# ray-project/ray_shuffling_data_loader

Hardware: AMD Instinct MI355X
Metric: shuffled_rows_per_sec (higher is better)
Workload: dtype bf16; 1 GPU; model=shuffling-data-loader + TabularMLP(100-512-256-128-1), global_batch=250000, rows_per_gpu=12500000, num_cols=100, batch_size_per_rank=250000, num_reducers=4, max_concurrent_epochs=2, parallelism=dp1, seed=0, burn_steps=0

## Files before the change

csrc/chain.h:

```cpp
#pragma once

#include <hip/hip_runtime.h>

#include <cstdint>

namespace rsdl {

struct ChainWeights {
  const void* W1;
  const float* b1;
  const void* W2;
  const float* b2;
  const void* W3;
  const float* b3;
  const void* w4;
  const float* b4;
};

struct FwdChainArgs {
  const void* x0s;
  ChainWeights w;
  void* a1t;
  uint32_t* mask1;
  void* a2t;
// ... 6 lines not shown
  int64_t M;
  int pi16, rows;
  int loss;
  bool weighted;
  const float* weight;
  float pos_weight;
};

struct EvalChainArgs {
  const void* x0s;
  ChainWeights w;
  float* pred;
  const float* target;
  float* part;
  int64_t M;
  int rows;
  int task;
  int64_t* hist;
  bool weighted;
  const float* weight;
};

struct BwdChainArgs {
  const void* dy;
  const void* a3;
  const void* mask1;
  const void* mask2;
  const void* w4;
  const void* W3T;
  const void* W2T;
  void* dz1t;
  void* dz2t;
  void* dz3t;
  float* db_part;
  int64_t M;
  int pi16, rows;
};

int64_t fwd_chain_grid(int64_t M, int rows);
void launch_swizzle_x(const void* x, void* out, int64_t M,
                      hipStream_t stream);
void launch_swizzle_xt(const void* x, void* out, int64_t M, int pi16,
                       hipStream_t stream);
void launch_swizzle_x_both(const void* x, void* xs, void* xt, int64_t M,
                           int pi16, hipStream_t stream);
void launch_fwd_chain(const FwdChainArgs& p, hipStream_t stream);
void launch_eval_chain(const EvalChainArgs& p, hipStream_t stream);

int64_t bwd_chain_grid(int64_t M, int rows);
void launch_bwd_chain(const BwdChainArgs& p, hipStream_t stream);

int64_t wgrad_frag_nslabs(int64_t mchunks, int32_t N, int32_t K,
                          int32_t nt_w, int32_t kt_w);
void launch_wgrad_frag(const void* AT, const void* BT, float* dW, int32_t N,
                       int32_t K, int64_t mchunks, int32_t nt_w,
                       int32_t kt_w, hipStream_t stream);
void launch_slab_reduce(const float* part, float* out, int64_t nk,
                        int64_t nslabs, hipStream_t stream);

}
```

csrc/shuffle_ops.cpp:

```cpp

#include <torch/extension.h>

#include <c10/hip/HIPStream.h>
#include <hip/hip_runtime.h>

#include <cmath>
#include <cstdlib>
#include <cstring>
#include <tuple>
#include <vector>

#include "chain.h"
#include "step_glue.h"

namespace rsdl {

enum DType : int32_t {
  DT_F32 = 0,
  DT_F64 = 1,
  DT_I32 = 2,
  DT_I64 = 3,
  DT_F16 = 4,
  DT_BF16 = 5,
  DT_U8 = 6,
// ... 816 lines not shown
              "bwd_chain: dy must be contiguous bf16 [M] or [M,1]");
  auto chk_a = [M](const at::Tensor& a, int64_t n, const char* nm) {
    TORCH_CHECK(a.is_cuda() && a.scalar_type() == at::kBFloat16 &&
                    a.dim() == 2 && a.size(0) == M && a.size(1) == n &&
                    a.is_contiguous(),
                "bwd_chain: ", nm, " must be contiguous bf16 [M,", n, "]");
  };
  chk_a(a3, 128, "a3");
  TORCH_CHECK(mask1.is_cuda() && mask1.scalar_type() == at::kInt &&
                  mask1.is_contiguous() && mask1.numel() == mtiles * 512,
              "bwd_chain: mask1 must be int32 [mtiles,512]");
  TORCH_CHECK(mask2.is_cuda() && mask2.scalar_type() == at::kInt &&
                  mask2.is_contiguous() && mask2.numel() == mtiles * 256,
              "bwd_chain: mask2 must be int32 [mtiles,256]");
  TORCH_CHECK(w4.numel() == 128 && w4.scalar_type() == at::kBFloat16,
              "bwd_chain: w4 must be bf16 [128]");
  TORCH_CHECK(W3.scalar_type() == at::kBFloat16 &&
                  ((W3.size(0) == 128 && W3.size(1) == 256) ||
                   (W3.size(0) == 256 && W3.size(1) == 128)),
              "bwd_chain: W3 must be bf16 [128,256] or W3^T [256,128]");
  TORCH_CHECK(W2.scalar_type() == at::kBFloat16 &&
                  ((W2.size(0) == 256 && W2.size(1) == 512) ||
                   (W2.size(0) == 512 && W2.size(1) == 256)),
              "bwd_chain: W2 must be bf16 [256,512] or W2^T [512,256]");
  auto w4c = w4.contiguous();
  auto W3Ts = (W3.size(0) == 128) ? swizzle_frag_T(W3.contiguous())
                                  : swizzle_frag(W3.contiguous());
  auto W2Ts = (W2.size(0) == 256) ? swizzle_frag_T(W2.contiguous())
                                  : swizzle_frag(W2.contiguous());
  auto bo = run_bwd_chain(dy, a3, mask1, mask2, w4c, W3Ts, W2Ts, pi16,
                          crows);
  auto& dz1t = bo.dz1t;
  auto& dz2t = bo.dz2t;
  auto& dz3t = bo.dz3t;
  auto& db_part = bo.db_part;
  auto db_full = at::zeros({kPartWPad}, dy.options().dtype(at::kFloat));
  launch_slab_reduce(db_part.data_ptr<float>(), db_full.data_ptr<float>(),
                     kPartWPad, db_part.size(0), current_stream());
  auto db = db_full.narrow(0, 0, kPartW);
  auto dw4 = (db.narrow(0, 897, 128) + db.narrow(0, 897 + 128, 128))
                 .reshape({1, 128});
  return {dz1t,
          dz2t,
          dz3t,
          db.narrow(0, 0, 512),
          db.narrow(0, 512, 256),
          db.narrow(0, 512 + 256, 128),
          db.narrow(0, 512 + 256 + 128, 1),
          dw4};
}

at::Tensor run_wgrad_frag(const at::Tensor& AT, const at::Tensor& BT,
                          int64_t N, int64_t K, int64_t mchunks,
                          int64_t nt_w, int64_t kt_w) {
  const int64_t nslabs = wgrad_frag_nslabs(mchunks, (int32_t)N, (int32_t)K,
                                           (int32_t)nt_w, (int32_t)kt_w);
  auto part = at::empty({nslabs, N * K}, AT.options().dtype(at::kFloat));
  launch_wgrad_frag(AT.data_ptr(), BT.data_ptr(), part.data_ptr<float>(),
                    (int32_t)N, (int32_t)K, mchunks, (int32_t)nt_w,
                    (int32_t)kt_w, current_stream());
  return part;
}

}
at::Tensor swizzle_xt_bf16(const at::Tensor& x, bool pi16) {
  check_x("swizzle_xt", x);
  const int64_t M = x.size(0);
  const int64_t mtiles = std::max<int64_t>((M + 31) / 32, 1);
  auto out = at::empty({4 * mtiles * 2 * 512}, x.options());
  if (M > 0) {
    launch_swizzle_xt(x.data_ptr(), out.data_ptr(), M, pi16 ? 1 : 0,
                      current_stream());
  }
  return out;
}

at::Tensor wgrad_frag_bf16(const at::Tensor& AT, const at::Tensor& BT,
                           int64_t N, int64_t K, int64_t mchunks,
                           int64_t nt_w, int64_t kt_w) {
  TORCH_CHECK(AT.is_cuda() && AT.scalar_type() == at::kBFloat16 &&
                  AT.is_contiguous() && BT.is_cuda() &&
                  BT.scalar_type() == at::kBFloat16 && BT.is_contiguous(),
              "wgrad_frag: inputs must be contiguous bf16 on GPU");
  TORCH_CHECK(AT.numel() == (N / 32) * mchunks * 512,
              "wgrad_frag: AT numel mismatch");
  TORCH_CHECK(BT.numel() == (K / 32) * mchunks * 512,
              "wgrad_frag: BT numel mismatch");
  TORCH_CHECK((nt_w == 2 && kt_w == 4) || (nt_w == 1 && kt_w == 8) ||
                  (nt_w == 1 && kt_w == 4),
              "wgrad_frag: unsupported tile config");
  TORCH_CHECK(N % (nt_w * 128) == 0 && K % (kt_w * 32) == 0,
              "wgrad_frag: N/K not divisible by block shape");
  auto dW = at::zeros({N, K}, AT.options().dtype(at::kFloat));
  if (mchunks > 0) {
    auto part = run_wgrad_frag(AT, BT, N, K, mchunks, nt_w, kt_w);
    const int64_t nslabs = part.size(0);
    launch_slab_reduce(part.data_ptr<float>(), dW.data_ptr<float>(),
                       N * K, nslabs, current_stream());
  }
  return dW;
}

namespace {

void check_master(const std::vector<at::Tensor>& w, const char* who) {
  TORCH_CHECK(w.size() == 4, who, ": weights must be [W1, W2, W3, w4]");
  const int64_t shp[4][2] = {{512, 100}, {256, 512}, {128, 256}, {1, 128}};
  for (int i = 0; i < 4; i++) {
    TORCH_CHECK(w[i].is_cuda() && w[i].scalar_type() == at::kFloat &&
                    w[i].is_contiguous() &&
                    w[i].numel() == shp[i][0] * shp[i][1] &&
                    (i == 3 || (w[i].dim() == 2 && w[i].size(0) == shp[i][0])),
                who, ": weight ", i, " must be contiguous fp32 [", shp[i][0],
                ",", shp[i][1], "] on GPU");
    TORCH_CHECK(reinterpret_cast<uintptr_t>(w[i].data_ptr()) % 16 == 0,
                who, ": weight ", i, " must be 16-byte aligned");
  }
}

struct PrepOut {
  at::Tensor W1s, W2s, W3s, W2Ts, W3Ts, w4b, tgt;
};

PrepOut run_step_prep(const std::vector<at::Tensor>& w,
                      const c10::optional<at::Tensor>& target,
                      const c10::optional<std::vector<at::Tensor>>& bufs) {
  check_master(w, "step_prep");
  const int64_t numel[6] = {512 * 112, 256 * 512, 128 * 256,
                            256 * 512, 128 * 256, 128};
  at::Tensor o[6];
  auto bf = w[0].options().dtype(at::kBFloat16);
  if (bufs.has_value()) {
    TORCH_CHECK(bufs->size() == 6, "step_prep: need six output buffers");
  }
  for (int i = 0; i < 6; i++) {
    if (bufs.has_value()) {
      o[i] = (*bufs)[i];
      TORCH_CHECK(o[i].is_cuda() && o[i].scalar_type() == at::kBFloat16 &&
                      o[i].is_contiguous() && o[i].numel() == numel[i] &&
                      reinterpret_cast<uintptr_t>(o[i].data_ptr()) % 16 == 0,
                  "step_prep: output buffer ", i,
                  " must be contiguous aligned bf16 with ", numel[i],
                  " elements");
    } else {
      o[i] = at::empty({numel[i]}, bf);
    }
  }
  PrepOut r{o[0], o[1], o[2], o[3], o[4], o[5], at::Tensor()};
  StepPrepArgs p{};
  p.W1 = w[0].data_ptr<float>();
  p.W2 = w[1].data_ptr<float>();
  p.W3 = w[2].data_ptr<float>();
  p.w4 = w[3].data_ptr<float>();
// ... 69 lines not shown
  }
  auto loss = at::empty({}, f32);
  StepFinArgs p{};
  p.part1 = part1.data_ptr<float>();
  p.part2 = part2.data_ptr<float>();
  p.part3 = part3.data_ptr<float>();
  p.db_part = db_part.data_ptr<float>();
  p.loss_part = loss_part.data_ptr<float>();
  p.ns1 = part1.size(0);
  p.ns2 = part2.size(0);
  p.ns3 = part3.size(0);
  p.db_rows = db_part.size(0);
  p.loss_n = loss_part.numel();
  p.M = M;
  p.dw1 = o[0].data_ptr<float>();
  p.dw2 = o[1].data_ptr<float>();
  p.dw3 = o[2].data_ptr<float>();
  p.dw4 = o[3].data_ptr<float>();
  p.db1 = o[4].data_ptr<float>();
  p.db2 = o[5].data_ptr<float>();
  p.db3 = o[6].data_ptr<float>();
  p.db4 = o[7].data_ptr<float>();
  p.loss = loss.data_ptr<float>();
  launch_step_finalize(p, current_stream());
  return {loss, o[0], o[1], o[2], o[3], o[4], o[5], o[6], o[7]};
}

}

std::vector<at::Tensor> step_prep(
    const std::vector<at::Tensor>& weights,
    const c10::optional<at::Tensor>& target,
    const c10::optional<std::vector<at::Tensor>>& outs) {
  auto r = run_step_prep(weights, target, outs);
  std::vector<at::Tensor> v = {r.W1s, r.W2s, r.W3s, r.W2Ts, r.W3Ts, r.w4b};
  if (target.has_value()) v.push_back(r.tgt);
  return v;
}

std::vector<at::Tensor> step_finalize(
    const at::Tensor& part1, const at::Tensor& part2,
    const at::Tensor& part3, const at::Tensor& db_part,
    const at::Tensor& loss_part, int64_t M,
    const c10::optional<std::vector<at::Tensor>>& outs) {
  return run_step_finalize(part1, part2, part3, db_part, loss_part, M, outs);
}

std::vector<at::Tensor> fused_step_bf16(
    const at::Tensor& x, const at::Tensor& target,
    const std::vector<at::Tensor>& weights,
    const std::vector<at::Tensor>& biases, bool pi16,
    const c10::optional<std::vector<at::Tensor>>& outs, int64_t rows,
    int64_t loss, const c10::optional<at::Tensor>& weight,
    double pos_weight) {
  const int crows = chain_rows(rows);
  const int closs = chain_loss(loss, "fused_step", "loss");
  const HeadWeights hw =
      head_weights("fused_step", x, weight, pos_weight, closs);
  check_x("fused_step", x);
  const int64_t M = x.size(0);
  TORCH_CHECK(M > 0, "fused_step: empty batch");
  TORCH_CHECK(target.numel() == M, "fused_step: target size mismatch");
  check_biases("fused_step", biases);
  auto pr = run_step_prep(weights, target, c10::nullopt);
  const int64_t mchunks = 2 * ((M + 31) / 32);
  c10::optional<at::Tensor> xt =
      at::empty({4 * mchunks * 512}, x.options());
  auto f = run_fwd_chain(x, pr.W1s, pr.W2s, pr.W3s, pr.w4b, biases[0],
                         biases[1], biases[2], biases[3], &pr.tgt, xt, pi16,
                         crows, closs, hw);
  auto b = run_bwd_chain(f.dyb, f.a3, f.mask1, f.mask2, pr.w4b, pr.W3Ts,
                         pr.W2Ts, pi16, crows);
  const char* st = std::getenv("RSDL_WGRAD_SMALL_TILES");
  const int64_t kt23 = (st != nullptr && std::strcmp(st, "1") == 0) ? 4 : 8;
  auto p1 = run_wgrad_frag(b.dz1t, *xt, 512, 128, mchunks, 2, 4);
  auto p2 = run_wgrad_frag(b.dz2t, f.a1t, 256, 512, mchunks, 1, kt23);
  auto p3 = run_wgrad_frag(b.dz3t, f.a2t, 128, 256, mchunks, 1, kt23);
  return run_step_finalize(p1, p2, p3, b.db_part, f.loss_part, M, outs);
}

std::tuple<c10::optional<at::Tensor>, c10::optional<at::Tensor>>
eval_chain_bf16(const at::Tensor& x, const std::vector<at::Tensor>& Wstage,
                const std::vector<at::Tensor>& biases,
                const c10::optional<at::Tensor>& target,
                const c10::optional<at::Tensor>& pred_out, bool want_pred,
                int64_t rows, int64_t task,
                const c10::optional<at::Tensor>& hist,
                const c10::optional<at::Tensor>& weight) {
  const int crows = chain_rows(rows);
  const int ctask = chain_loss(task, "eval_chain", "task");
  check_x("eval_chain", x);
  const int64_t M = x.size(0);
  TORCH_CHECK(Wstage.size() == 4,
              "eval_chain: Wstage must be [W1s, W2s, W3s, w4b]");
  const int64_t wn[4] = {512 * 112, 256 * 512, 128 * 256, 128};
  for (int i = 0; i < 4; i++) {
    TORCH_CHECK(Wstage[i].is_cuda() &&
                    Wstage[i].scalar_type() == at::kBFloat16 &&
                    Wstage[i].is_contiguous() && Wstage[i].numel() == wn[i] &&
                    Wstage[i].get_device() == x.get_device() &&
                    reinterpret_cast<uintptr_t>(Wstage[i].data_ptr()) % 16 ==
                        0,
                "eval_chain: staged weight ", i,
                " must be contiguous aligned bf16 with ", wn[i],
                " elements on x's GPU");
  }
  check_biases("eval_chain", biases, x.get_device());
  const bool with_pred = want_pred || pred_out.has_value();
  TORCH_CHECK(with_pred || target.has_value(),
              "eval_chain: nothing to compute (no target, no predictions)");
  at::Tensor tgt, pred, part;
  if (target.has_value()) {
    TORCH_CHECK(target->is_cuda() &&
                    target->get_device() == x.get_device() &&
                    (target->scalar_type() == at::kFloat ||
                     target->scalar_type() == at::kDouble),
                "eval_chain: target must be fp32 or fp64 on x's GPU");
    TORCH_CHECK(target->numel() == M, "eval_chain: target size mismatch");
    tgt = target->reshape({-1}).to(at::kFloat).contiguous();
  }
  if (pred_out.has_value()) {
    TORCH_CHECK(pred_out->is_cuda() &&
                    pred_out->get_device() == x.get_device() &&
                    pred_out->scalar_type() == at::kFloat &&
                    pred_out->is_contiguous() && pred_out->numel() == M,
                "eval_chain: pred_out must be contiguous fp32 with ", M,
                " elements on x's GPU");
    pred = *pred_out;
  } else if (with_pred) {
    pred = at::empty({M}, x.options().dtype(at::kFloat));
// ... 50 lines not shown
                     int64_t M) {
  TORCH_CHECK(part.is_cuda() && part.scalar_type() == at::kFloat &&
                  part.is_contiguous() && part.dim() == 2 &&
                  (part.size(1) == 4 || part.size(1) == 8) &&
                  reinterpret_cast<uintptr_t>(part.data_ptr()) % 16 == 0,
              "eval_accumulate: part must be contiguous aligned fp32 [n,4] "
              "(or [n,8], weighted) on GPU");
  const bool wide = part.size(1) == 8;
  TORCH_CHECK(acc.is_cuda() && acc.scalar_type() == at::kDouble &&
                  acc.is_contiguous() && acc.numel() == (wide ? 6 : 5) &&
                  acc.get_device() == part.get_device(),
              "eval_accumulate: acc must be contiguous fp64 [",
              wide ? 6 : 5, "] on part's GPU");
  TORCH_CHECK(M >= 0, "eval_accumulate: M must not be negative");
  launch_eval_accumulate(part.data_ptr<float>(), part.size(0), M,
                         acc.data_ptr<double>(), wide ? 5 : 4,
                         current_stream());
}

}

PYBIND11_MODULE(TORCH_EXTENSION_NAME, m) {
  m.doc() = "MI355X (gfx950) fused shuffle kernels";
  m.def("gather_rows", &rsdl::gather_rows, "row gather of packed rows",
        py::arg("src"), py::arg("perm"));
  m.def("gather_rows_out", &rsdl::gather_rows_out, py::arg("src"),
        py::arg("perm"), py::arg("dst"));
  m.def("unpack_permute", &rsdl::unpack_permute, py::arg("packed"),
        py::arg("perm"), py::arg("outs"), py::arg("packed_offsets"),
        py::arg("src_dtype_codes"));
  m.def("unpack_permute_affine", &rsdl::unpack_permute_affine,
        py::arg("packed"), py::arg("perm"), py::arg("outs"),
        py::arg("packed_offsets"), py::arg("src_dtype_codes"),
        py::arg("aff_table"), py::arg("aff_base"),
        py::arg("nan_fill") = c10::nullopt);
  m.def("column_stats", &rsdl::column_stats, py::arg("packed"),
        py::arg("packed_offsets"), py::arg("src_dtype_codes"),
        py::arg("numels"));
  m.def("pack_columns", &rsdl::pack_columns, py::arg("cols"),
        py::arg("packed_offsets"), py::arg("packed_dtype_codes"),
        py::arg("row_stride"), py::arg("perm") = c10::nullopt);
  m.def("pack_columns_tiled", &rsdl::pack_columns_tiled, py::arg("cols"),
        py::arg("packed_offsets"), py::arg("packed_dtype_codes"),
        py::arg("row_stride"), py::arg("out") = c10::nullopt);
  m.def("partition_build_perm", &rsdl::partition_build_perm, py::arg("dest"),
        py::arg("num_dests"));
  m.def("wgrad_bf16", &rsdl::wgrad_bf16, py::arg("dy"), py::arg("x"),
        py::arg("with_bias") = true);
  m.def("relu_bwd_bias", &rsdl::relu_bwd_bias, py::arg("dy"), py::arg("y"));
  m.def("swizzle_xt_bf16", &rsdl::swizzle_xt_bf16, py::arg("x"),
        py::arg("pi16") = false);
  m.def("wgrad_frag_bf16", &rsdl::wgrad_frag_bf16, py::arg("AT"),
        py::arg("BT"), py::arg("N"), py::arg("K"), py::arg("mchunks"),
        py::arg("nt_w"), py::arg("kt_w"));
  m.def("fwd_chain_bf16", &rsdl::fwd_chain_bf16, py::arg("x"),
        py::arg("W1"), py::arg("b1"), py::arg("W2"), py::arg("b2"),
        py::arg("W3"), py::arg("b3"), py::arg("w4"), py::arg("b4"),
        py::arg("target") = c10::nullopt,
        py::arg("xt_out") = c10::nullopt, py::arg("pi16") = false,
        py::arg("rows") = 0, py::arg("loss") = 0,
        py::arg("weight") = c10::nullopt, py::arg("pos_weight") = 1.0);
  m.def("bwd_chain_bf16", &rsdl::bwd_chain_bf16, py::arg("dy"),
        py::arg("a3"), py::arg("mask1"), py::arg("mask2"), py::arg("w4"),
        py::arg("W3"), py::arg("W2"), py::arg("pi16") = false,
        py::arg("rows") = 0);
  m.def("step_prep", &rsdl::step_prep, py::arg("weights"),
        py::arg("target") = c10::nullopt, py::arg("outs") = c10::nullopt);
  m.def("step_finalize", &rsdl::step_finalize, py::arg("part1"),
        py::arg("part2"), py::arg("part3"), py::arg("db_part"),
        py::arg("loss_part"), py::arg("M"), py::arg("outs") = c10::nullopt);
  m.def("fused_step_bf16", &rsdl::fused_step_bf16, py::arg("x"),
        py::arg("target"), py::arg("weights"), py::arg("biases"),
        py::arg("pi16") = false, py::arg("outs") = c10::nullopt,
        py::arg("rows") = 0, py::arg("loss") = 0,
        py::arg("weight") = c10::nullopt, py::arg("pos_weight") = 1.0);
  m.def("eval_chain_bf16", &rsdl::eval_chain_bf16, py::arg("x"),
        py::arg("Wstage"), py::arg("biases"),
        py::arg("target") = c10::nullopt, py::arg("pred_out") = c10::nullopt,
        py::arg("want_pred") = true, py::arg("rows") = 0,
        py::arg("task") = 0, py::arg("hist") = c10::nullopt,
        py::arg("weight") = c10::nullopt);
  m.def("eval_accumulate", &rsdl::eval_accumulate, py::arg("part"),
        py::arg("acc"), py::arg("M"));
  m.attr("LOSS_MSE") = (int)rsdl::kLossMse;
  m.attr("LOSS_BCE") = (int)rsdl::kLossBce;
  m.attr("HEAD_WEIGHTS") = 1;
  m.attr("DT_F32") = (int)rsdl::DT_F32;
  m.attr("DT_F64") = (int)rsdl::DT_F64;
  m.attr("DT_I32") = (int)rsdl::DT_I32;
  m.attr("DT_I64") = (int)rsdl::DT_I64;
  m.attr("DT_F16") = (int)rsdl::DT_F16;
  m.attr("DT_BF16") = (int)rsdl::DT_BF16;
  m.attr("DT_U8") = (int)rsdl::DT_U8;
}
```

csrc/wgrad_frag.hip:

```cpp

#include <hip/hip_runtime.h>
#include <hip/hip_bf16.h>

#include <cstdint>
#include <cstdlib>

#include "chain.h"

namespace rsdl {

typedef __attribute__((__vector_size__(8 * sizeof(short)))) short wf_bf16x8;
typedef __attribute__((__vector_size__(16 * sizeof(float)))) float wf_f32x16;

template <int NT_W, int KT_W, int MIN_WAVES = 2, int SCHED = 0>
__global__ void __launch_bounds__(256, MIN_WAVES) wgrad_frag_kernel(
    const short* __restrict__ AT, const short* __restrict__ BT,
    float* __restrict__ dW,
    int32_t N, int32_t K, int64_t mchunks, int32_t nblk_n, int32_t nblk_k,
    int64_t nslabs, int64_t chunks_per_slab) {
  const int32_t NBLK = (nblk_n < 0 ? -nblk_n : nblk_n) * nblk_k;
  int64_t slab;
  int32_t blk;
  if (nblk_n < 0) {
    nblk_n = -nblk_n;
// ... 92 lines not shown
    if (i + 2 < iters) WF_MFMA(a2, b2);
    if (i + 3 < iters) WF_MFMA(a0, b0);
  } else if (SCHED2) {
    WF_LOAD(a0, b0, 0);
    WF_LOAD(a1, b1, 1);
    while (i + 4 <= iters) {
      WF_FENCE();
      WF_MFMA(a0, b0);
      WF_FENCE();
      WF_LOAD(a0, b0, i + 2);
      WF_FENCE();
      WF_MFMA(a1, b1);
      WF_FENCE();
      WF_LOAD(a1, b1, i + 3);
      WF_FENCE();
      i += 2;
    }
    if (i + 2 < iters) WF_LOAD(a2, b2, i + 2);
    if (i < iters) WF_MFMA(a0, b0);
    if (i + 1 < iters) WF_MFMA(a1, b1);
    if (i + 2 < iters) WF_MFMA(a2, b2);
  } else {
    while (i + 3 <= iters) {
      WF_LOAD(a2, b2, i + 2);
      WF_MFMA(a0, b0);
      if (i + 3 < iters) WF_LOAD(a0, b0, i + 3);
      WF_MFMA(a1, b1);
      if (i + 4 < iters) WF_LOAD(a1, b1, i + 4);
      WF_MFMA(a2, b2);
      i += 3;
    }
    if (i < iters) WF_MFMA(a0, b0);
    if (i + 1 < iters) WF_MFMA(a1, b1);
  }
#undef WF_LOAD
#undef WF_MFMA
#undef WF_FENCE

  float* part = dW + slab * (int64_t)N * K;
  #pragma unroll
  for (int nt = 0; nt < NT_W; nt++) {
    #pragma unroll
    for (int kt = 0; kt < KT_W; kt++) {
      const int32_t k = (kt0 + kt) * 32 + (lane & 31);
      #pragma unroll
      for (int reg = 0; reg < 16; reg++) {
        const int32_t n = (nt0 + nt) * 32 + (reg & 3) + 8 * (reg >> 2) +
                          4 * (lane >> 5);
        part[(int64_t)n * K + k] = acc[nt][kt][reg];
      }
    }
  }
}

typedef __attribute__((__vector_size__(4 * sizeof(float)))) float wf_f32x4;
template <int SCHED = 0>
__global__ void __launch_bounds__(256) slab_reduce_kernel(
    const float* __restrict__ part, float* __restrict__ out, int64_t nk4,
    int64_t nslabs, int64_t s1) {
  const int64_t i = (int64_t)blockIdx.x * 256 + threadIdx.x;
  if (i >= nk4) return;
  const int64_t lo = (int64_t)blockIdx.y * s1;
  const int64_t hi = min(lo + s1, nslabs);
  wf_f32x4 s0 = {0.f, 0.f, 0.f, 0.f}, s1v = s0, s2 = s0, s3 = s0;
  int64_t sl = lo;
  if (SCHED) {
    wf_f32x4 la[4], lb[4];
#define SR_LOAD(buf, base)                                                 \
  {                                                                        \
    _Pragma("unroll") for (int j = 0; j < 4; j++) {                        \
      buf[j] = *reinterpret_cast<const wf_f32x4*>(                         \
          part + (((base) + j) * nk4 + i) * 4);                            \
    }                                                                      \
  }
#define SR_ACC(buf)                                                        \
  {                                                                        \
    s0 += buf[0];                                                          \
    s1v += buf[1];                                                         \
    s2 += buf[2];                                                          \
    s3 += buf[3];                                                          \
  }
    if (sl + 4 <= hi) {
      SR_LOAD(la, sl);
      while (sl + 12 <= hi) {
        SR_LOAD(lb, sl + 4);
        __builtin_amdgcn_sched_barrier(0);
        SR_ACC(la);
        __builtin_amdgcn_sched_barrier(0);
        SR_LOAD(la, sl + 8);
        __builtin_amdgcn_sched_barrier(0);
        SR_ACC(lb);
        __builtin_amdgcn_sched_barrier(0);
        sl += 8;
      }
      if (sl + 8 <= hi) {
        SR_LOAD(lb, sl + 4);
        SR_ACC(la);
        SR_ACC(lb);
        sl += 8;
      } else {
        SR_ACC(la);
        sl += 4;
      }
    }
#undef SR_LOAD
#undef SR_ACC
// ... 10 lines not shown
      s0 += l0;
      s1v += l1;
      s2 += l2;
      s3 += l3;
    }
  }
  for (; sl < hi; sl++) {
    s0 += *reinterpret_cast<const wf_f32x4*>(part + (sl * nk4 + i) * 4);
  }
  const wf_f32x4 s = (s0 + s1v) + (s2 + s3);
  float* o = out + i * 4;
  unsafeAtomicAdd(&o[0], s[0]);
  unsafeAtomicAdd(&o[1], s[1]);
  unsafeAtomicAdd(&o[2], s[2]);
  unsafeAtomicAdd(&o[3], s[3]);
}

void launch_slab_reduce(const float* part, float* out, int64_t nk,
                        int64_t nslabs, hipStream_t stream) {
  const int64_t nk4 = nk / 4;
  const int64_t gx = (nk4 + 255) / 256;
  int64_t nsplit = (512 + gx - 1) / gx;
  if (nsplit > nslabs) nsplit = nslabs;
  const int64_t s1 = (nslabs + nsplit - 1) / nsplit;
  nsplit = (nslabs + s1 - 1) / s1;
  static bool sched = [] {
    const char* e = std::getenv("RSDL_WGRAD_SCHED");
    return e && e[0] == '1';
  }();
  auto kern = sched ? slab_reduce_kernel<1> : slab_reduce_kernel<0>;
  hipLaunchKernelGGL(kern,
                     dim3((uint32_t)gx, (uint32_t)nsplit), dim3(256), 0,
                     stream, part, out, nk4, nslabs, s1);
}

static int64_t frag_target(int32_t K, int32_t nt_w) {
  static int64_t env_target = [] {
    const char* e = std::getenv("RSDL_WGRAD_WGS");
    return e ? atoll(e) : 0;
  }();
  if (env_target > 0) return env_target;
  return (nt_w == 2) ? 256 : (K >= 512 ? 512 : 256);
}

int64_t wgrad_frag_nslabs(int64_t mchunks, int32_t N, int32_t K,
                          int32_t nt_w, int32_t kt_w) {
  const int32_t nblk = (N / (nt_w * 128)) * (K / (kt_w * 32));
  int64_t nslabs = (frag_target(K, nt_w) + nblk - 1) / nblk;
  if (nslabs > mchunks) nslabs = mchunks;
  const int64_t cps = (mchunks + nslabs - 1) / nslabs;
  return (mchunks + cps - 1) / cps;
}

void launch_wgrad_frag(const void* AT, const void* BT, float* dW, int32_t N,
                       int32_t K, int64_t mchunks, int32_t nt_w,
                       int32_t kt_w, hipStream_t stream) {
  const int32_t nblk_n = N / (nt_w * 128);
  const int32_t nblk_k = K / (kt_w * 32);
  const int32_t nblk = nblk_n * nblk_k;
  int64_t target = frag_target(K, nt_w);
  int64_t nslabs = (target + nblk - 1) / nblk;
  if (nslabs > mchunks) nslabs = mchunks;
  const int64_t chunks_per_slab = (mchunks + nslabs - 1) / nslabs;
  nslabs = (mchunks + chunks_per_slab - 1) / chunks_per_slab;
  static bool linear = std::getenv("RSDL_WGRAD_LINEAR") != nullptr;
  static bool sched = [] {
    const char* e = std::getenv("RSDL_WGRAD_SCHED");
    return e && e[0] == '1';
  }();
  const int64_t grid =
      linear ? nslabs * nblk : ((nslabs + 7) / 8) * 8 * nblk;
  const int32_t nb_n = linear ? -nblk_n : nblk_n;
  if (nt_w == 2 && kt_w == 4) {
    auto kern = sched ? wgrad_frag_kernel<2, 4, 2, 1>
                      : wgrad_frag_kernel<2, 4>;
    hipLaunchKernelGGL(kern, dim3((uint32_t)grid),
                       dim3(256), 0, stream,
                       reinterpret_cast<const short*>(AT),
                       reinterpret_cast<const short*>(BT), dW, N, K, mchunks,
                       nb_n, nblk_k, nslabs, chunks_per_slab);
  } else if (nt_w == 1 && kt_w == 8) {
    auto kern = sched ? wgrad_frag_kernel<1, 8, 2, 1>
                      : wgrad_frag_kernel<1, 8>;
    hipLaunchKernelGGL(kern, dim3((uint32_t)grid),
                       dim3(256), 0, stream,
                       reinterpret_cast<const short*>(AT),
                       reinterpret_cast<const short*>(BT), dW, N, K, mchunks,
                       nb_n, nblk_k, nslabs, chunks_per_slab);
  } else if (nt_w == 1 && kt_w == 4) {
    auto kern = sched ? wgrad_frag_kernel<1, 4, 3, 1>
                      : wgrad_frag_kernel<1, 4, 3>;
    hipLaunchKernelGGL(kern, dim3((uint32_t)grid),
                       dim3(256), 0, stream,
                       reinterpret_cast<const short*>(AT),
                       reinterpret_cast<const short*>(BT), dW, N, K, mchunks,
                       nb_n, nblk_k, nslabs, chunks_per_slab);
  }
}

}
```

ray_shuffling_data_loader_amd/models/fused_step.py:

```python

import os
from typing import Tuple

import torch

from ray_shuffling_data_loader_amd.models.mlp import TabularMLP

_PI16 = os.environ.get("RSDL_PI16", "0") == "1"

_CHAIN_ROWS = int(os.environ.get("RSDL_CHAIN_ROWS", "0") or "0")

_NATIVE_GLUE = os.environ.get("RSDL_NATIVE_GLUE", "1") != "0"


def _layers(model: TabularMLP):
    lin = [m for m in model.modules() if isinstance(m, torch.nn.Linear)]
    assert len(lin) == 4, "fused_step requires the stock TabularMLP(100)"
    shapes = [(512, 100), (256, 512), (128, 256), (1, 128)]
    for m, (n, k) in zip(lin, shapes):
        assert m.weight.shape == (n, k), (m.weight.shape, (n, k))
    return lin


def _weight_buffers(model: TabularMLP, lin):
    buf = getattr(model, "_fused_buf", None)
    dev = lin[0].weight.device
    if buf is None or buf["W1p"].device != dev:
        bf = dict(dtype=torch.bfloat16, device=dev)
        buf = {
            "W1p": torch.zeros(512, 112, **bf),
            "W2": torch.empty(256, 512, **bf),
            "W3": torch.empty(128, 256, **bf),
            "w4": torch.empty(128, **bf),
        }
        model._fused_buf = buf
    torch._foreach_copy_(
        [buf["W1p"][:, :100], buf["W2"], buf["W3"], buf["w4"]],
        [
            lin[0].weight.detach(),
            lin[1].weight.detach(),
            lin[2].weight.detach(),
            lin[3].weight.detach().view(-1),
        ],
    )
    return buf


_LOSSES = {"mse": 0, "bce": 1}


def _loss_kw(code: int) -> dict:
    return {"loss": code} if code else {}


def loss_head(out: torch.Tensor, target: torch.Tensor, m_rows: int,
              loss: str = "bce", sample_weight=None, pos_weight=None):
    o = out.float().reshape(-1, 1)
    t = target.float().reshape(-1, 1).to(o.device)
    inv_m = torch.tensor(1.0 / m_rows, dtype=torch.float32, device=o.device)
    if sample_weight is None:
        w = torch.ones_like(o)
    else:
        w = sample_weight.float().reshape(-1, 1).to(o.device)
# ... 9 lines not shown
        term = torch.clamp(o, min=0.0) - o * t + torch.log1p(e)
    else:
        pt = float(pos_weight) * t
        lp = torch.log1p(e)
        term = (pt * (torch.clamp(-o, min=0.0) + lp)
                + (1.0 - t) * (torch.clamp(o, min=0.0) + lp))
        g = (1.0 - t) * sg - pt * torch.where(o >= 0, small, big)
    dyb = ((inv_m * w) * g).bfloat16()
    return dyb, (w * term).sum().reshape(1)


def bce_head(out: torch.Tensor, target: torch.Tensor, m_rows: int):
    return loss_head(out, target, m_rows)


def _head_args(M: int, loss: str, sample_weight, pos_weight):
    if pos_weight is not None:
        if loss != "bce":
            raise ValueError(
                "fused_step: pos_weight needs loss='bce', got "
                f"loss={loss!r}")
        pos_weight = float(pos_weight)
        if not (pos_weight > 0.0 and pos_weight != float("inf")):
            raise ValueError(
                "fused_step: pos_weight must be finite and > 0, got "
                f"{pos_weight!r}")
        if pos_weight == 1.0:
            pos_weight = None
    if sample_weight is not None:
        if sample_weight.numel() != M:
            raise ValueError(
                f"fused_step: sample_weight has {sample_weight.numel()} "
                f"values for {M} rows")
        sample_weight = sample_weight.reshape(-1)
        if sample_weight.dtype != torch.float32:
            sample_weight = sample_weight.float()
        sample_weight = sample_weight.contiguous()
    return sample_weight, pos_weight


def _weight_kw(sample_weight, pos_weight) -> dict:
    kw = {}
    if sample_weight is not None:
        kw["weight"] = sample_weight
    if pos_weight is not None:
        kw["pos_weight"] = pos_weight
    return kw


def _rows_kw() -> dict:
    return {"rows": _CHAIN_ROWS} if _CHAIN_ROWS else {}


def _native_ok(hip, lin, x, target, grad_hook) -> bool:
    if not (_NATIVE_GLUE and grad_hook is None
            and hasattr(hip, "fused_step_bf16")):
        return False
    if not (x.is_cuda and x.dtype == torch.bfloat16 and x.dim() == 2
            and x.shape[0] > 0 and x.is_contiguous()):
        return False
    if not (target.is_cuda and target.numel() == x.shape[0]
            and target.dtype in (torch.float32, torch.float64)):
        return False
    return all(
        p.is_cuda and p.dtype == torch.float32 and p.is_contiguous()
        and p.data_ptr() % 16 == 0
        for m in lin for p in (m.weight, m.bias)
    )


def _flat_outs(lin):
    outs = [m.weight.grad for m in lin] + [m.bias.grad for m in lin]
    for i, g in enumerate(outs):
        if g is None or g.dtype != torch.float32 or not g.is_contiguous():
            return None
        if i < 3 and g.data_ptr() % 16 != 0:
            return None
    return outs


def fused_step(
    model: TabularMLP, x: torch.Tensor, target: torch.Tensor,
    grad_hook=None, loss: str = "mse", sample_weight=None,
    pos_weight=None,
) -> Tuple[torch.Tensor, None]:
    if loss not in _LOSSES:
        raise ValueError(
            f"fused_step: loss must be 'mse' or 'bce', got {loss!r}")
    loss_code = _LOSSES[loss]
    M = x.shape[0]
    loss_name = loss
    sample_weight, pos_weight = _head_args(M, loss, sample_weight,
                                           pos_weight)
    weighted = sample_weight is not None or pos_weight is not None
    from ray_shuffling_data_loader_amd.ops.shuffle_ops import _load_hip

    hip = _load_hip()
    lin = _layers(model)
    has_weights = bool(getattr(hip, "HEAD_WEIGHTS", 0))
    from ray_shuffling_data_loader_amd.ops.shuffle_ops import wgrad_frag

    if _native_ok(hip, lin, x, target, grad_hook) and (
            not weighted or (has_weights and (
                sample_weight is None or sample_weight.device == x.device))):
        flat_mode = getattr(model, "_rsdl_flat_grads", False)
        outs = _flat_outs(lin) if flat_mode else None
        if not flat_mode or outs is not None:
            res = hip.fused_step_bf16(
                x, target,
                [m.weight.detach() for m in lin],
                [m.bias.detach() for m in lin],
                pi16=_PI16, outs=outs, **_rows_kw(), **_loss_kw(loss_code),
                **_weight_kw(sample_weight, pos_weight),
            )
            if outs is None:
                for i, m in enumerate(lin):
                    m.weight.grad = res[1 + i]
                    m.bias.grad = res[5 + i]
            return res[0]

    buf = _weight_buffers(model, lin)
    b1, b2, b3, b4 = (m.bias.detach() for m in lin)
    mchunks = 2 * ((M + 31) // 32)
    xt = torch.empty(4 * mchunks * 512, dtype=torch.bfloat16,
                     device=x.device)
    if (loss_code and not hasattr(hip, "LOSS_BCE")) or (
            weighted and not has_weights):
        a1t, mask1, a2t, mask2, a3, out = hip.fwd_chain_bf16(
            x, buf["W1p"], b1, buf["W2"], b2, buf["W3"], b3, buf["w4"], b4,
            target=None, xt_out=xt, pi16=_PI16, **_rows_kw(),
        )
        dyb, loss_part = loss_head(out, target, M, loss_name,
                                   sample_weight, pos_weight)
    else:
        a1t, mask1, a2t, mask2, a3, out, dyb, loss_part = (
            hip.fwd_chain_bf16(
                x, buf["W1p"], b1, buf["W2"], b2, buf["W3"], b3, buf["w4"],
                b4, target=target, xt_out=xt, pi16=_PI16, **_rows_kw(),
                **_loss_kw(loss_code),
                **_weight_kw(
                    None if sample_weight is None
                    else sample_weight.to(x.device),
                    pos_weight),
            )
        )
    loss = loss_part.sum() / M
    dz1t, dz2t, dz3t, db1, db2, db3, db4, dw4 = hip.bwd_chain_bf16(
        dyb, a3, mask1, mask2, buf["w4"], buf["W3"], buf["W2"], pi16=_PI16,
        **_rows_kw(),
    )
    flat_mode = getattr(model, "_rsdl_flat_grads", False)
    if flat_mode and grad_hook is not None:
        for m, gb in zip(lin, (db1, db2, db3, db4)):
            m.bias.grad.copy_(gb.reshape(m.bias.shape))
        lin[3].weight.grad.copy_(dw4)
        grad_hook("bias")
    dw1 = wgrad_frag(dz1t, xt, 512, 128, mchunks)[:, :100].contiguous()
    if flat_mode and grad_hook is not None:
        lin[0].weight.grad.copy_(dw1)
        grad_hook("w1")
    dw2 = wgrad_frag(dz2t, a1t, 256, 512, mchunks)
    if flat_mode and grad_hook is not None:
        lin[1].weight.grad.copy_(dw2)
        grad_hook("w2")
    dw3 = wgrad_frag(dz3t, a2t, 128, 256, mchunks)
    if flat_mode and grad_hook is not None:
        lin[2].weight.grad.copy_(dw3)
        grad_hook("w3")
        return loss
    grads = [
        (dw1, db1),
        (dw2, db2),
        (dw3, db3),
        (dw4, db4),
    ]
    for m, (gw, gb) in zip(lin, grads):
        gb = gb.reshape(m.bias.shape)
        if flat_mode:
            m.weight.grad.copy_(gw)
            m.bias.grad.copy_(gb)
        else:
            m.weight.grad = gw.to(m.weight.dtype)
            m.bias.grad = gb.to(m.bias.dtype)
    return loss
```

ray_shuffling_data_loader_amd/ops/shuffle_ops.py:

```python

from typing import Dict, List, NamedTuple, Optional, Sequence, Tuple, Union

import os

import numpy as np
import torch

from ray_shuffling_data_loader_amd.utils.schema import (
    Schema,
    TORCH_TO_NUMPY_DTYPE,
)

_hip = None
_hip_err = None


def _load_hip():
    global _hip, _hip_err
    if _hip is None and _hip_err is None:
        try:
            from ray_shuffling_data_loader_amd import _rsdl_hip

            _hip = _rsdl_hip
        except ImportError as e:
# ... 370 lines not shown
    num_dests: int,
):
    if packed.is_cuda:
        hip = _load_hip()
        perm, counts = hip.partition_build_perm(dest, num_dests)
        grouped = gather_rows(packed, perm)
        return grouped, counts
    counts = torch.bincount(dest, minlength=num_dests)
    order = torch.argsort(dest, stable=True)
    grouped = gather_rows(packed, order)
    return grouped, counts




def wgrad(dy: torch.Tensor, x: torch.Tensor, with_bias: bool = True):
    if dy.is_cuda and dy.dtype == torch.bfloat16 and x.dtype == torch.bfloat16:
        hip = _load_hip()
        dw, db = hip.wgrad_bf16(dy.contiguous(), x.contiguous(), with_bias)
        return dw, (db if with_bias else None)
    dw = dy.t().float() @ x.float()
    db = dy.float().sum(0) if with_bias else None
    return dw, db


_PI16_IDX = [(p & 3) | ((p & 4) << 1) | ((p & 8) >> 1) for p in range(16)]


def t_frag_swizzle(t: torch.Tensor, pi16: bool = False) -> torch.Tensor:
    m, c = t.shape
    mp = (m + 15) // 16 * 16
    if mp != m:
        t = torch.nn.functional.pad(t, (0, 0, 0, mp - m))
    v = t.reshape(mp // 16, 16, c)
    if pi16:
        v = v[:, _PI16_IDX]
    v = v.reshape(mp // 16, 2, 8, c // 32, 32)
    return v.permute(3, 0, 1, 4, 2).contiguous().reshape(-1)


_WGRAD_FRAG_CFG = {
    (512, 128): (2, 4),
    (256, 512): (1, 8),
    (128, 256): (1, 8),
}
_WGRAD_FRAG_SMALL = {
    (512, 128): (2, 4),
    (256, 512): (1, 4),
    (128, 256): (1, 4),
}


def wgrad_frag(at_frag: torch.Tensor, bt_frag: torch.Tensor, n: int,
               k: int, mchunks: int) -> torch.Tensor:
    cfg = (
        _WGRAD_FRAG_SMALL
        if os.environ.get("RSDL_WGRAD_SMALL_TILES", "0") == "1"
        else _WGRAD_FRAG_CFG
    )
    nt_w, kt_w = cfg[(n, k)]
    hip = _load_hip()
    return hip.wgrad_frag_bf16(at_frag, bt_frag, n, k, mchunks, nt_w, kt_w)


def t_frag_unswizzle(
    flat: torch.Tensor, m: int, c: int, pi16: bool = False
) -> torch.Tensor:
    mchunks = flat.numel() // (c * 16)
    v = flat.reshape(c // 32, mchunks, 2, 32, 8)
    v = v.permute(1, 2, 4, 0, 3).reshape(mchunks, 16, c)
    if pi16:
        v = v[:, _PI16_IDX]
    return v.reshape(mchunks * 16, c)[:m].contiguous()


def relu_mask_words(a: torch.Tensor) -> torch.Tensor:
    m, n = a.shape
    mt = (m + 31) // 32
    pad = mt * 32 - m
    bits = a > 0
    if pad:
        bits = torch.cat(
            [bits, torch.zeros(pad, n, dtype=torch.bool, device=a.device)]
        )
    bits = bits.view(mt, 32, n).long()
    weights = (1 << torch.arange(32, device=a.device, dtype=torch.long))
    words = (bits * weights.view(1, 32, 1)).sum(1)
    return (words & 0xFFFFFFFF).to(torch.int32) if False else (
        words - ((words >> 31) & 1) * (1 << 32)
    ).to(torch.int32)
```

Before: 306.1 million rows/s.

## Add LDS ring-buffered wgrad kernel with async global-to-LDS loads

Adds a wgrad kernel that streams A/B fragments into a six-stage shared-memory ring using global_load_lds, with vmcnt waits and barriers so loads for later chunks overlap the MFMA work on the current one. By default it is used for the dW2 and dW3 tile configs (1x8), but not dW1 or the scheduled variant. Environment and variant arguments allow forcing either path. Costs are a large LDS footprint that limits occupancy, plus per-iteration barriers.

```diff
diff --git a/csrc/chain.h b/csrc/chain.h
--- a/csrc/chain.h
+++ b/csrc/chain.h
@@ -82,9 +82,10 @@
 
 int64_t wgrad_frag_nslabs(int64_t mchunks, int32_t N, int32_t K,
                           int32_t nt_w, int32_t kt_w);
+bool wgrad_frag_has_lds(int32_t nt_w, int32_t kt_w);
 void launch_wgrad_frag(const void* AT, const void* BT, float* dW, int32_t N,
                        int32_t K, int64_t mchunks, int32_t nt_w,
-                       int32_t kt_w, hipStream_t stream);
+                       int32_t kt_w, int32_t variant, hipStream_t stream);
 void launch_slab_reduce(const float* part, float* out, int64_t nk,
                         int64_t nslabs, hipStream_t stream);
 
diff --git a/csrc/shuffle_ops.cpp b/csrc/shuffle_ops.cpp
--- a/csrc/shuffle_ops.cpp
+++ b/csrc/shuffle_ops.cpp
@@ -892,32 +892,19 @@
 
 at::Tensor run_wgrad_frag(const at::Tensor& AT, const at::Tensor& BT,
                           int64_t N, int64_t K, int64_t mchunks,
-                          int64_t nt_w, int64_t kt_w) {
+                          int64_t nt_w, int64_t kt_w, int64_t variant) {
   const int64_t nslabs = wgrad_frag_nslabs(mchunks, (int32_t)N, (int32_t)K,
                                            (int32_t)nt_w, (int32_t)kt_w);
   auto part = at::empty({nslabs, N * K}, AT.options().dtype(at::kFloat));
   launch_wgrad_frag(AT.data_ptr(), BT.data_ptr(), part.data_ptr<float>(),
                     (int32_t)N, (int32_t)K, mchunks, (int32_t)nt_w,
-                    (int32_t)kt_w, current_stream());
+                    (int32_t)kt_w, (int32_t)variant, current_stream());
   return part;
 }
 
-}
-at::Tensor swizzle_xt_bf16(const at::Tensor& x, bool pi16) {
-  check_x("swizzle_xt", x);
-  const int64_t M = x.size(0);
-  const int64_t mtiles = std::max<int64_t>((M + 31) / 32, 1);
-  auto out = at::empty({4 * mtiles * 2 * 512}, x.options());
-  if (M > 0) {
-    launch_swizzle_xt(x.data_ptr(), out.data_ptr(), M, pi16 ? 1 : 0,
-                      current_stream());
-  }
-  return out;
-}
-
-at::Tensor wgrad_frag_bf16(const at::Tensor& AT, const at::Tensor& BT,
-                           int64_t N, int64_t K, int64_t mchunks,
-                           int64_t nt_w, int64_t kt_w) {
+void check_wgrad_frag(const at::Tensor& AT, const at::Tensor& BT, int64_t N,
+                      int64_t K, int64_t mchunks, int64_t nt_w, int64_t kt_w,
+                      int64_t variant) {
   TORCH_CHECK(AT.is_cuda() && AT.scalar_type() == at::kBFloat16 &&
                   AT.is_contiguous() && BT.is_cuda() &&
                   BT.scalar_type() == at::kBFloat16 && BT.is_contiguous(),
@@ -931,14 +918,49 @@
               "wgrad_frag: unsupported tile config");
   TORCH_CHECK(N % (nt_w * 128) == 0 && K % (kt_w * 32) == 0,
               "wgrad_frag: N/K not divisible by block shape");
+  TORCH_CHECK(variant >= 0 && variant <= 2,
+              "wgrad_frag: variant must be 0 (default), 1 (direct) or 2 "
+              "(LDS ring), got ", variant);
+  TORCH_CHECK(variant != 2 ||
+                  wgrad_frag_has_lds((int32_t)nt_w, (int32_t)kt_w),
+              "wgrad_frag: no LDS-ring kernel for tile config (", nt_w, ",",
+              kt_w, ")");
+}
+
+}
+at::Tensor swizzle_xt_bf16(const at::Tensor& x, bool pi16) {
+  check_x("swizzle_xt", x);
+  const int64_t M = x.size(0);
+  const int64_t mtiles = std::max<int64_t>((M + 31) / 32, 1);
+  auto out = at::empty({4 * mtiles * 2 * 512}, x.options());
+  if (M > 0) {
+    launch_swizzle_xt(x.data_ptr(), out.data_ptr(), M, pi16 ? 1 : 0,
+                      current_stream());
+  }
+  return out;
+}
+
+at::Tensor wgrad_frag_bf16(const at::Tensor& AT, const at::Tensor& BT,
+                           int64_t N, int64_t K, int64_t mchunks,
+                           int64_t nt_w, int64_t kt_w, int64_t variant) {
+  check_wgrad_frag(AT, BT, N, K, mchunks, nt_w, kt_w, variant);
   auto dW = at::zeros({N, K}, AT.options().dtype(at::kFloat));
   if (mchunks > 0) {
-    auto part = run_wgrad_frag(AT, BT, N, K, mchunks, nt_w, kt_w);
+    auto part = run_wgrad_frag(AT, BT, N, K, mchunks, nt_w, kt_w, variant);
     const int64_t nslabs = part.size(0);
     launch_slab_reduce(part.data_ptr<float>(), dW.data_ptr<float>(),
                        N * K, nslabs, current_stream());
   }
   return dW;
+}
+
+at::Tensor wgrad_frag_partials_bf16(const at::Tensor& AT,
+                                    const at::Tensor& BT, int64_t N,
+                                    int64_t K, int64_t mchunks, int64_t nt_w,
+                                    int64_t kt_w, int64_t variant) {
+  check_wgrad_frag(AT, BT, N, K, mchunks, nt_w, kt_w, variant);
+  TORCH_CHECK(mchunks > 0, "wgrad_frag_partials: mchunks must be positive");
+  return run_wgrad_frag(AT, BT, N, K, mchunks, nt_w, kt_w, variant);
 }
 
 namespace {
@@ -1114,9 +1136,12 @@
     const std::vector<at::Tensor>& biases, bool pi16,
     const c10::optional<std::vector<at::Tensor>>& outs, int64_t rows,
     int64_t loss, const c10::optional<at::Tensor>& weight,
-    double pos_weight) {
+    double pos_weight, int64_t wgrad_variant) {
   const int crows = chain_rows(rows);
   const int closs = chain_loss(loss, "fused_step", "loss");
+  TORCH_CHECK(wgrad_variant >= 0 && wgrad_variant <= 2,
+              "fused_step: wgrad_variant must be 0, 1 or 2, got ",
+              wgrad_variant);
   const HeadWeights hw =
       head_weights("fused_step", x, weight, pos_weight, closs);
   check_x("fused_step", x);
@@ -1135,9 +1160,10 @@
                          pr.W2Ts, pi16, crows);
   const char* st = std::getenv("RSDL_WGRAD_SMALL_TILES");
   const int64_t kt23 = (st != nullptr && std::strcmp(st, "1") == 0) ? 4 : 8;
-  auto p1 = run_wgrad_frag(b.dz1t, *xt, 512, 128, mchunks, 2, 4);
-  auto p2 = run_wgrad_frag(b.dz2t, f.a1t, 256, 512, mchunks, 1, kt23);
-  auto p3 = run_wgrad_frag(b.dz3t, f.a2t, 128, 256, mchunks, 1, kt23);
+  const int64_t wv = wgrad_variant;
+  auto p1 = run_wgrad_frag(b.dz1t, *xt, 512, 128, mchunks, 2, 4, wv);
+  auto p2 = run_wgrad_frag(b.dz2t, f.a1t, 256, 512, mchunks, 1, kt23, wv);
+  auto p3 = run_wgrad_frag(b.dz3t, f.a2t, 128, 256, mchunks, 1, kt23, wv);
   return run_step_finalize(p1, p2, p3, b.db_part, f.loss_part, M, outs);
 }
 
@@ -1294,7 +1320,11 @@
         py::arg("pi16") = false);
   m.def("wgrad_frag_bf16", &rsdl::wgrad_frag_bf16, py::arg("AT"),
         py::arg("BT"), py::arg("N"), py::arg("K"), py::arg("mchunks"),
-        py::arg("nt_w"), py::arg("kt_w"));
+        py::arg("nt_w"), py::arg("kt_w"), py::arg("variant") = 0);
+  m.def("wgrad_frag_partials_bf16", &rsdl::wgrad_frag_partials_bf16,
+        py::arg("AT"), py::arg("BT"), py::arg("N"), py::arg("K"),
+        py::arg("mchunks"), py::arg("nt_w"), py::arg("kt_w"),
+        py::arg("variant") = 0);
   m.def("fwd_chain_bf16", &rsdl::fwd_chain_bf16, py::arg("x"),
         py::arg("W1"), py::arg("b1"), py::arg("W2"), py::arg("b2"),
         py::arg("W3"), py::arg("b3"), py::arg("w4"), py::arg("b4"),
@@ -1315,7 +1345,8 @@
         py::arg("target"), py::arg("weights"), py::arg("biases"),
         py::arg("pi16") = false, py::arg("outs") = c10::nullopt,
         py::arg("rows") = 0, py::arg("loss") = 0,
-        py::arg("weight") = c10::nullopt, py::arg("pos_weight") = 1.0);
+        py::arg("weight") = c10::nullopt, py::arg("pos_weight") = 1.0,
+        py::arg("wgrad_variant") = 0);
   m.def("eval_chain_bf16", &rsdl::eval_chain_bf16, py::arg("x"),
         py::arg("Wstage"), py::arg("biases"),
         py::arg("target") = c10::nullopt, py::arg("pred_out") = c10::nullopt,
diff --git a/csrc/wgrad_frag.hip b/csrc/wgrad_frag.hip
--- a/csrc/wgrad_frag.hip
+++ b/csrc/wgrad_frag.hip
@@ -168,6 +168,140 @@
     }
   }
 }
+
+constexpr int kLdsStages = 6;
+constexpr int kLdsStageElems = 12 * 512;
+
+#define WL_WAIT(n) \
+  asm volatile("s_waitcnt vmcnt(" #n ") lgkmcnt(0)" ::: "memory")
+
+template <int NT_W, int KT_W>
+__global__ void __launch_bounds__(256, 2) wgrad_lds_kernel(
+    const short* __restrict__ AT, const short* __restrict__ BT,
+    float* __restrict__ dW,
+    int32_t N, int32_t K, int64_t mchunks, int32_t nblk_n, int32_t nblk_k,
+    int64_t nslabs, int64_t chunks_per_slab) {
+  constexpr int S = kLdsStages;
+  constexpr int P = S - 1;
+  constexpr int NA = 4 * NT_W;
+  static_assert(NA + KT_W == 12, "a stage is 12 fragments, 3 per wave");
+  static_assert(P - 1 == 4, "WL_WAIT counts below assume S == 6");
+  __shared__ __attribute__((aligned(16))) short ring[S * kLdsStageElems];
+
+  const int32_t NBLK = (nblk_n < 0 ? -nblk_n : nblk_n) * nblk_k;
+  int64_t slab;
+  int32_t blk;
+  if (nblk_n < 0) {
+    nblk_n = -nblk_n;
+    blk = (int32_t)(blockIdx.x % (uint32_t)NBLK);
+    slab = blockIdx.x / (uint32_t)NBLK;
+  } else {
+    const int32_t xcd = blockIdx.x & 7;
+    const int32_t g = blockIdx.x >> 3;
+    blk = g % NBLK;
+    slab = (int64_t)(g / NBLK) * 8 + xcd;
+  }
+  if (slab >= nslabs) return;
+  const int32_t bn = blk / nblk_k;
+  const int32_t bk = blk % nblk_k;
+  const int64_t c0 = slab * chunks_per_slab;
+  const int64_t cend = min(c0 + chunks_per_slab, mchunks);
+  if (c0 >= cend) return;
+  const int64_t iters = cend - c0;
+
+  const int32_t wave = __builtin_amdgcn_readfirstlane(threadIdx.x >> 6);
+  const int32_t lane = threadIdx.x & 63;
+  const int32_t nt0 = bn * NA + wave * NT_W;
+  const int32_t kt0 = bk * KT_W;
+
+  const short* gp[3];
+  #pragma unroll
+  for (int j = 0; j < 3; j++) {
+    const int32_t f = wave * 3 + j;
+    const short* base =
+        f < NA ? AT + ((int64_t)(bn * NA + f) * mchunks + c0) * 512
+               : BT + ((int64_t)(kt0 + f - NA) * mchunks + c0) * 512;
+    gp[j] = base + lane * 8;
+  }
+
+  wf_f32x16 acc[NT_W][KT_W] = {};
+
+#define WL_ISSUE(st)                                                       \
+  {                                                                        \
+    _Pragma("unroll") for (int j = 0; j < 3; j++) {                        \
+      __builtin_amdgcn_global_load_lds(                                    \
+          (const __attribute__((address_space(1))) void*)gp[j],            \
+          (__attribute__((address_space(3))) void*)(                       \
+              ring + (st) * kLdsStageElems + (wave * 3 + j) * 512),        \
+          16, 0, 0);                                                       \
+      gp[j] += 512;                                                        \
+    }                                                                      \
+  }
+#define WL_CONSUME(st)                                                     \
+  {                                                                        \
+    const short* sp = ring + (st) * kLdsStageElems + lane * 8;             \
+    wf_bf16x8 a[NT_W], b[KT_W];                                            \
+    _Pragma("unroll") for (int nt = 0; nt < NT_W; nt++) {                  \
+      a[nt] = *reinterpret_cast<const wf_bf16x8*>(                         \
+          sp + (wave * NT_W + nt) * 512);                                  \
+    }                                                                      \
+    _Pragma("unroll") for (int kt = 0; kt < KT_W; kt++) {                  \
+      b[kt] = *reinterpret_cast<const wf_bf16x8*>(sp + (NA + kt) * 512);   \
+    }                                                                      \
+    _Pragma("unroll") for (int nt = 0; nt < NT_W; nt++) {                  \
+      _Pragma("unroll") for (int kt = 0; kt < KT_W; kt++) {                \
+        acc[nt][kt] = __builtin_amdgcn_mfma_f32_32x32x16_bf16(             \
+            a[nt], b[kt], acc[nt][kt], 0, 0, 0);                           \
+      }                                                                    \
+    }                                                                      \
+  }
+
+  int32_t ws = 0, rs = 0;
+  const int64_t pre = iters < P ? iters : P;
+  for (int64_t j = 0; j < pre; j++) {
+    WL_ISSUE(ws);
+    ws = ws + 1 == S ? 0 : ws + 1;
+  }
+  int64_t i = 0;
+  for (; i + P < iters; i++) {
+    WL_WAIT(12);
+    __builtin_amdgcn_s_barrier();
+    WL_ISSUE(ws);
+    ws = ws + 1 == S ? 0 : ws + 1;
+    WL_CONSUME(rs);
+    rs = rs + 1 == S ? 0 : rs + 1;
+  }
+  for (; i < iters; i++) {
+    switch (iters - 1 - i) {
+      case 0: WL_WAIT(0); break;
+      case 1: WL_WAIT(3); break;
+      case 2: WL_WAIT(6); break;
+      case 3: WL_WAIT(9); break;
+      default: WL_WAIT(12); break;
+    }
+    __builtin_amdgcn_s_barrier();
+    WL_CONSUME(rs);
+    rs = rs + 1 == S ? 0 : rs + 1;
+  }
+#undef WL_ISSUE
+#undef WL_CONSUME
+
+  float* part = dW + slab * (int64_t)N * K;
+  #pragma unroll
+  for (int nt = 0; nt < NT_W; nt++) {
+    #pragma unroll
+    for (int kt = 0; kt < KT_W; kt++) {
+      const int32_t k = (kt0 + kt) * 32 + (lane & 31);
+      #pragma unroll
+      for (int reg = 0; reg < 16; reg++) {
+        const int32_t n = (nt0 + nt) * 32 + (reg & 3) + 8 * (reg >> 2) +
+                          4 * (lane >> 5);
+        part[(int64_t)n * K + k] = acc[nt][kt][reg];
+      }
+    }
+  }
+}
+#undef WL_WAIT
 
 typedef __attribute__((__vector_size__(4 * sizeof(float)))) float wf_f32x4;
 template <int SCHED = 0>
@@ -284,9 +418,40 @@
   return (mchunks + cps - 1) / cps;
 }
 
+#ifndef RSDL_WGRAD_LDS_DEFAULT_DW1
+#define RSDL_WGRAD_LDS_DEFAULT_DW1 0
+#endif
+#ifndef RSDL_WGRAD_LDS_DEFAULT_DW2
+#define RSDL_WGRAD_LDS_DEFAULT_DW2 1
+#endif
+#ifndef RSDL_WGRAD_LDS_DEFAULT_DW3
+#define RSDL_WGRAD_LDS_DEFAULT_DW3 1
+#endif
+
+bool wgrad_frag_has_lds(int32_t nt_w, int32_t kt_w) {
+  return (nt_w == 2 && kt_w == 4) || (nt_w == 1 && kt_w == 8);
+}
+
+static bool wgrad_use_lds(int32_t variant, int32_t K, int32_t nt_w,
+                          int32_t kt_w, bool sched) {
+  if (!wgrad_frag_has_lds(nt_w, kt_w)) return false;
+  if (variant != 0) return variant == 2;
+  static const int env = [] {
+    const char* e = std::getenv("RSDL_WGRAD_LDS");
+    return (e != nullptr && (e[0] == '0' || e[0] == '1') && e[1] == '\0')
+               ? e[0] - '0'
+               : -1;
+  }();
+  if (env >= 0) return env == 1;
+  if (sched) return false;
+  if (nt_w == 2) return RSDL_WGRAD_LDS_DEFAULT_DW1 != 0;
+  return (K >= 512 ? RSDL_WGRAD_LDS_DEFAULT_DW2
+                   : RSDL_WGRAD_LDS_DEFAULT_DW3) != 0;
+}
+
 void launch_wgrad_frag(const void* AT, const void* BT, float* dW, int32_t N,
                        int32_t K, int64_t mchunks, int32_t nt_w,
-                       int32_t kt_w, hipStream_t stream) {
+                       int32_t kt_w, int32_t variant, hipStream_t stream) {
   const int32_t nblk_n = N / (nt_w * 128);
   const int32_t nblk_k = K / (kt_w * 32);
   const int32_t nblk = nblk_n * nblk_k;
@@ -303,7 +468,13 @@
   const int64_t grid =
       linear ? nslabs * nblk : ((nslabs + 7) / 8) * 8 * nblk;
   const int32_t nb_n = linear ? -nblk_n : nblk_n;
-  if (nt_w == 2 && kt_w == 4) {
+  if (wgrad_use_lds(variant, K, nt_w, kt_w, sched)) {
+    auto kern = nt_w == 2 ? wgrad_lds_kernel<2, 4> : wgrad_lds_kernel<1, 8>;
+    hipLaunchKernelGGL(kern, dim3((uint32_t)grid), dim3(256), 0, stream,
+                       reinterpret_cast<const short*>(AT),
+                       reinterpret_cast<const short*>(BT), dW, N, K, mchunks,
+                       nb_n, nblk_k, nslabs, chunks_per_slab);
+  } else if (nt_w == 2 && kt_w == 4) {
     auto kern = sched ? wgrad_frag_kernel<2, 4, 2, 1>
                       : wgrad_frag_kernel<2, 4>;
     hipLaunchKernelGGL(kern, dim3((uint32_t)grid),
diff --git a/ray_shuffling_data_loader_amd/models/fused_step.py b/ray_shuffling_data_loader_amd/models/fused_step.py
--- a/ray_shuffling_data_loader_amd/models/fused_step.py
+++ b/ray_shuffling_data_loader_amd/models/fused_step.py
@@ -9,6 +9,8 @@
 _PI16 = os.environ.get("RSDL_PI16", "0") == "1"
 
 _CHAIN_ROWS = int(os.environ.get("RSDL_CHAIN_ROWS", "0") or "0")
+
+_WGRAD_VARIANT = 0
 
 _NATIVE_GLUE = os.environ.get("RSDL_NATIVE_GLUE", "1") != "0"
 
@@ -124,6 +126,10 @@
     return {"rows": _CHAIN_ROWS} if _CHAIN_ROWS else {}
 
 
+def _wgrad_kw() -> dict:
+    return {"wgrad_variant": _WGRAD_VARIANT} if _WGRAD_VARIANT else {}
+
+
 def _native_ok(hip, lin, x, target, grad_hook) -> bool:
     if not (_NATIVE_GLUE and grad_hook is None
             and hasattr(hip, "fused_step_bf16")):
@@ -183,7 +189,7 @@
                 [m.weight.detach() for m in lin],
                 [m.bias.detach() for m in lin],
                 pi16=_PI16, outs=outs, **_rows_kw(), **_loss_kw(loss_code),
-                **_weight_kw(sample_weight, pos_weight),
+                **_weight_kw(sample_weight, pos_weight), **_wgrad_kw(),
             )
             if outs is None:
                 for i, m in enumerate(lin):
@@ -227,15 +233,15 @@
             m.bias.grad.copy_(gb.reshape(m.bias.shape))
         lin[3].weight.grad.copy_(dw4)
         grad_hook("bias")
-    dw1 = wgrad_frag(dz1t, xt, 512, 128, mchunks)[:, :100].contiguous()
+    dw1 = wgrad_frag(dz1t, xt, 512, 128, mchunks, _WGRAD_VARIANT)[:, :100].contiguous()
     if flat_mode and grad_hook is not None:
         lin[0].weight.grad.copy_(dw1)
         grad_hook("w1")
-    dw2 = wgrad_frag(dz2t, a1t, 256, 512, mchunks)
+    dw2 = wgrad_frag(dz2t, a1t, 256, 512, mchunks, _WGRAD_VARIANT)
     if flat_mode and grad_hook is not None:
         lin[1].weight.grad.copy_(dw2)
         grad_hook("w2")
-    dw3 = wgrad_frag(dz3t, a2t, 128, 256, mchunks)
+    dw3 = wgrad_frag(dz3t, a2t, 128, 256, mchunks, _WGRAD_VARIANT)
     if flat_mode and grad_hook is not None:
         lin[2].weight.grad.copy_(dw3)
         grad_hook("w3")
diff --git a/ray_shuffling_data_loader_amd/ops/shuffle_ops.py b/ray_shuffling_data_loader_amd/ops/shuffle_ops.py
--- a/ray_shuffling_data_loader_amd/ops/shuffle_ops.py
+++ b/ray_shuffling_data_loader_amd/ops/shuffle_ops.py
@@ -446,7 +446,7 @@
 
 
 def wgrad_frag(at_frag: torch.Tensor, bt_frag: torch.Tensor, n: int,
-               k: int, mchunks: int) -> torch.Tensor:
+               k: int, mchunks: int, variant: int = 0) -> torch.Tensor:
     cfg = (
         _WGRAD_FRAG_SMALL
         if os.environ.get("RSDL_WGRAD_SMALL_TILES", "0") == "1"
@@ -454,7 +454,9 @@
     )
     nt_w, kt_w = cfg[(n, k)]
     hip = _load_hip()
-    return hip.wgrad_frag_bf16(at_frag, bt_frag, n, k, mchunks, nt_w, kt_w)
+    kw = {"variant": variant} if variant else {}
+    return hip.wgrad_frag_bf16(at_frag, bt_frag, n, k, mchunks, nt_w, kt_w,
+                               **kw)
 
 
 def t_frag_unswizzle(
```

New measurement: 330.3 million rows/s, median of 6. 1.08x the previous value.
